# B-R-P/NMSLIB-ZIG

Hardware: AMD Instinct MI355X
Metric: queries/sec @ recall@10, 1M x 128-D L2, batch=1024; HBM GB/s vs peak (higher is better)
Workload: dtype f16+f32

## Files before the change

### nmslib_zig_amd/csrc/kernels/bf_kernels.hip

```cpp
#include <cstdio>
#include <type_traits>
#include <vector>
#include <cstdlib>

#include "common_dev.hpp"
#include "kernels.hpp"

namespace gfxknn {

enum BfMode : int { BF_L2 = 0, BF_DOT = 1, BF_COS = 2, BF_L1 = 3, BF_LINF = 4, BF_COSC = 5, BF_L2D = 6 };

struct BfArgs {
    const float* base;
    const float* aux;
    const float* qaux;
    int aux_stride;
    const float* queries;
    u64* cand;
    int* cand_cnt;
    uint32_t* gthr;
    uint32_t* gq;
    int xj, xm;
    int n, ldb, nqt, nsplit, rows_per_split, kprime, cap;
    int kcs;
// ... 772 lines not shown
        else asm volatile("s_waitcnt vmcnt(0)\n\ts_barrier" ::: "memory");
    }
    if (nstages > 0 && !(a.dbg & 1)) {
        if (a.xj > 0 && !(a.dbg & 256)) exchange_counted();
        finish_stage(true);
    }
    if (h == 0) a.cand_cnt[(size_t)qidx * a.nsplit + split] = mycnt;
}

__device__ __forceinline__ uint32_t hit_mask_f32(const f32x16& c, float t) {
    typedef float f32x2 __attribute__((ext_vector_type(2)));
    uint32_t m = 0u;
    const f32x2 tt = {t, t};
#pragma unroll
    for (int i0 = 0; i0 < 16; i0 += 8) {
        f32x2 d[4];
#pragma unroll
        for (int j = 0; j < 4; ++j) d[j] = f32x2{c[i0 + 2 * j], c[i0 + 2 * j + 1]} - tt;
        asm volatile("" : "+v"(d[0]), "+v"(d[1]), "+v"(d[2]), "+v"(d[3]));
#pragma unroll
        for (int j = 0; j < 4; ++j) {
            m = __builtin_amdgcn_alignbit(m, __float_as_uint(d[j][0]), 31);
            m = __builtin_amdgcn_alignbit(m, __float_as_uint(d[j][1]), 31);
        }
    }
    return ~m & 0xffffu;
}
__device__ __forceinline__ uint32_t hit_mask_i32(const i32x16& c, int t) {
    uint32_t m = 0u;
#pragma unroll
    for (int i = 0; i < 16; ++i) m = __builtin_amdgcn_alignbit(m, (uint32_t)(c[i] - t), 31);
    return ~m & 0xffffu;
}
__device__ __forceinline__ void scan_gather_entries(u64* keys, const int* offs, const uint32_t* list, int q, int nl, int caph,
                                                    int tps, int tid, int nthreads) {
    for (int s = tid; s < nl; s += nthreads) {
        const int len = offs[s + 1] - offs[s];
        if (len == 0) continue;
        const uint32_t* e = list + (size_t)q * caph * nl + s;
        const uint32_t row_base = (uint32_t)(s >> 1) * (uint32_t)tps * BF_BN + 4u * (s & 1);
        uint32_t pre[4];
#pragma unroll
        for (int i = 0; i < 4; ++i) pre[i] = (i < len && i < caph) ? e[(size_t)i * nl] : 0u;
        int j = 0;
        auto expand = [&](const uint32_t ent) __attribute__((always_inline)) {
            uint32_t m = ent & 0xffffu;
            const uint32_t r0 = row_base + (ent >> 16) * 32u;
            while (m && j < len) {
                const int bit = 31 - __builtin_clz(m);
                m &= ~(1u << bit);
                const int reg = 15 - bit;
                keys[offs[s] + j++] = (u64)(r0 + (reg & 3) + 8 * (reg >> 2));
            }
        };
#pragma unroll
        for (int i = 0; i < 4; ++i)
            if (i < caph && j < len) expand(pre[i]);
        for (int i = 4; i < caph && j < len; ++i) expand(e[(size_t)i * nl]);
    }
}

struct BfScanArgs {
    const uint8_t* base_i8;
    const int32_t* auxh;
    const uint8_t* queries;
    const int* thr;
    uint32_t* list;
    int* list_cnt;
    int n, nqt, nsplit, tps, caph;
    int tile_stride;
    int* top8;
};

template <int QG, bool SAMPLE>
__global__ __launch_bounds__(256, 2) void bf_scan_u8_kernel(BfScanArgs a) {
    extern __shared__ __attribute__((aligned(16))) char smem[];
    const int tid = threadIdx.x, lane = tid & 63, wave = tid >> 6;
    const int h = lane >> 5, l31 = lane & 31;
    const int b = blockIdx.x;
    const int xcd = b & 7, rest = b >> 3;
    const int qt = rest % a.nqt;
    const int split = (rest / a.nqt) * 8 + xcd;
    if (split >= a.nsplit) return;

    constexpr int kGroup = 4, kRing = 2 * kGroup, kAuxRing = 8, kTileBytes = BF_BN * 128;
    char* ring = smem;
    int* auxr = reinterpret_cast<int*>(ring + kRing * kTileBytes);

    const int tstr = SAMPLE ? a.tile_stride : 1;
    const int tiles_all = (a.n + BF_BN - 1) / BF_BN;
    const int stiles_all = (tiles_all + tstr - 1) / tstr;
// ... 1073 lines not shown
        const float need = 2.1f * e1;
        uint32_t best = 0u;
#pragma unroll
        for (int i = 0; i < NPER; ++i) {
            const float v = ord_f32(key[i]);
            const bool c = key[i] != 0u && key[i] <= T && v > -INFINITY && t3 - v >= need;
            best = c && key[i] > best ? key[i] : best;
        }
#pragma unroll
        for (int o = 32; o > 0; o >>= 1) {
            const uint32_t other = (uint32_t)__shfl_xor((int)best, o, 64);
            best = other > best ? other : best;
        }
        ok = false;
        if (best != 0u) {
            int above = 0;
#pragma unroll
            for (int i = 0; i < NPER; ++i) above += __popcll(__builtin_amdgcn_ballot_w64(key[i] > best));
            const int jmax = rcap < total ? rcap : total;
            const int j = best == T ? r : above + 1;
            if (j <= jmax) {
                t1 = ord_f32(best);
                ok = true;
            }
        }
    }
    if (lane == 0) {
        thr3[q] = (t3 - 1.02f * e1) / unit;
        thr1[q] = force_precise == 2 ? INFINITY : t1;
        if (!ok) atomicOr(&precise[q / group_q], 1);
    }
}

struct RerankListF32Args {
    const float* base;
    const float* queries;
    const uint32_t* list;
    const int* list_cnt;
    const int32_t* ext_ids;
    int32_t* out_ids;
    float* out_dists;
    int32_t* out_cnt;
    int* tile_fail;
    int n, k, nsplit, caph, p2max, fail_queries, space, dim, ldb;
    int tps;
    const float* queries_sel;
    const float* thr;
    const float* thr1;
    const int* precise;
    int no_split;
    float bmax;
    float bres;
    float scale, scale_q, bres16;
    int sel_dim, sel_ld;
    const float* qaux;
    unsigned long long* prof;
};

__global__ __launch_bounds__(256) void bf_rerank_f32_list_kernel(RerankListF32Args a) {
    const unsigned long long t0 = a.prof ? wall_clock64() : 0;
    auto lap = [&](int i) __attribute__((always_inline)) {
        if (a.prof && threadIdx.x == 0) atomicAdd(&a.prof[i], wall_clock64() - t0);
    };
    extern __shared__ __attribute__((aligned(16))) char smem[];
    u64* keys = reinterpret_cast<u64*>(smem);
    int* offs = reinterpret_cast<int*>(keys + a.p2max);
    __shared__ int s_over, s_split;
    __shared__ float s_qn2, s_e1, s_thr;
    const int q = blockIdx.x, tid = threadIdx.x, lane = tid & 63, wave = tid >> 6;
    const int nl = 2 * a.nsplit;
    if (tid == 0) s_over = 0;
    __syncthreads();
    if (tid < 64) {
        const int per = (nl + 63) / 64;
        int sum = 0, over = 0;
        for (int i = 0; i < per; ++i) {
            const int s = tid * per + i;
            if (s < nl) {
                const int c = a.list_cnt[(size_t)q * nl + s];
                over |= c > a.caph;
                sum += c < a.caph ? c : a.caph;
            }
        }
        int incl = sum;
#pragma unroll
        for (int o = 1; o < 64; o <<= 1) {
            const int v = __shfl_up(incl, o, 64);
            if (tid >= o) incl += v;
        }
        int run = incl - sum;
        for (int i = 0; i < per; ++i) {
// ... 41 lines not shown
    if (a.prof && tid == 0) {
        atomicAdd(&a.prof[8], (unsigned long long)total);
        atomicAdd(&a.prof[9], (unsigned long long)P);
        atomicAdd(&a.prof[10], 1ull);
    }
    const float* qq = a.queries + (size_t)q * a.ldb;
    const int sub = lane & 15, rg = lane >> 4;
    if (a.dim <= 128) {
        float qv[8];
        bool ok[8];
    #pragma unroll
        for (int c = 0; c < 8; ++c) {
            const int d = sub + 16 * c;
            ok[c] = d < a.dim;
            qv[c] = ok[c] ? qq[d] : 0.f;
        }
        constexpr int kU = 4;
        for (int j0 = wave * (4 * kU); j0 < total; j0 += 16 * kU) {
            uint32_t pos[kU];
            float xv[kU][8];
    #pragma unroll
            for (int u = 0; u < kU; ++u) {
                const int j = j0 + 4 * u + rg;
                pos[u] = (uint32_t)keys[j < total ? j : total - 1];
                const float* row = a.base + (size_t)pos[u] * a.ldb + sub;
    #pragma unroll
                for (int c = 0; c < 8; ++c) xv[u][c] = ok[c] ? row[16 * c] : 0.f;
            }
            __builtin_amdgcn_wave_barrier();
    #pragma unroll
            for (int u = 0; u < kU; ++u) {
                float p0[4], p1[4], p2[4];
    #pragma unroll
                for (int v = 0; v < 4; ++v) {
                    p0[v] = p1[v] = p2[v] = 0.f;
    #pragma unroll
                    for (int c = 0; c < 2; ++c) {
                        if (64 * c >= a.dim) continue;
                        const float x = xv[u][v + 4 * c], y = qv[v + 4 * c];
                        if (a.space == SP_L2) {
                            const float t = x - y;
                            p0[v] = fmaf(t, t, p0[v]);
                        } else {
                            p0[v] = fmaf(x, y, p0[v]);
                            if (a.space != SP_NEGDOT) {
                                p1[v] = fmaf(x, x, p1[v]);
                                p2[v] = fmaf(y, y, p2[v]);
                            }
                        }
                    }
                }
                auto tree = [&](const float* p) __attribute__((always_inline)) -> float {
                    float s = (p[0] + p[2]) + (p[1] + p[3]);
    #pragma unroll
                    for (int o = 8; o > 0; o >>= 1) s += __shfl_xor(s, o, 64);
                    return s;
                };
                const float s0 = tree(p0);
                float d;
                if (a.space == SP_L2) d = sqrtf(s0);
                else if (a.space == SP_NEGDOT) d = -s0;
                else {
                    const float sim = normdot_finish(s0, tree(p1), tree(p2));
                    d = a.space == SP_ANGULAR ? acosf(sim) : fmaxf(0.0f, 1.0f - sim);
                }
                const int j = j0 + 4 * u + rg;
                if (sub == 0 && j < total) keys[j] = ((u64)f32_ord(d) << 32) | pos[u];
            }
        }
    } else {
        const int nstep = (a.dim + 63) >> 6;
        for (int j0 = wave * 16; j0 < total; j0 += 64) {
            uint32_t pos[4];
            const float* rowp[4];
    #pragma unroll
            for (int u = 0; u < 4; ++u) {
                const int j = j0 + 4 * u + rg;
                pos[u] = (uint32_t)keys[j < total ? j : total - 1];
                rowp[u] = a.base + (size_t)pos[u] * a.ldb + sub;
            }
            float p0[4][4], p1[4][4], p2[4][4];
    #pragma unroll
            for (int u = 0; u < 4; ++u)
    #pragma unroll
                for (int v = 0; v < 4; ++v) p0[u][v] = p1[u][v] = p2[u][v] = 0.f;
            for (int c0 = 0; c0 < nstep; c0 += 2) {
                float xv[4][8], qv[8];
                bool ok[8];
    #pragma unroll
                for (int c = 0; c < 8; ++c) {
                    const int d = sub + 16 * (c & 3) + 64 * (c0 + (c >> 2));
                    ok[c] = d < a.dim;
                    qv[c] = ok[c] ? qq[d] : 0.f;
    #pragma unroll
                    for (int u = 0; u < 4; ++u) xv[u][c] = ok[c] ? rowp[u][16 * (c & 3) + 64 * (c0 + (c >> 2))] : 0.f;
                }
    #pragma unroll
                for (int u = 0; u < 4; ++u) {
    #pragma unroll
                    for (int v = 0; v < 4; ++v) {
    #pragma unroll
                        for (int c = 0; c < 2; ++c) {
                            if (64 * (c0 + c) >= a.dim) continue;
                            const float x = xv[u][v + 4 * c], y = qv[v + 4 * c];
                            if (a.space == SP_L2) {
                                const float t = x - y;
                                p0[u][v] = fmaf(t, t, p0[u][v]);
                            } else {
                                p0[u][v] = fmaf(x, y, p0[u][v]);
                                if (a.space != SP_NEGDOT) {
                                    p1[u][v] = fmaf(x, x, p1[u][v]);
                                    p2[u][v] = fmaf(y, y, p2[u][v]);
                                }
                            }
                        }
                    }
                }
            }
            __builtin_amdgcn_wave_barrier();
    #pragma unroll
            for (int u = 0; u < 4; ++u) {
                auto tree = [&](const float* p) __attribute__((always_inline)) -> float {
                    float s = (p[0] + p[2]) + (p[1] + p[3]);
    #pragma unroll
                    for (int o = 8; o > 0; o >>= 1) s += __shfl_xor(s, o, 64);
                    return s;
                };
                const float s0 = tree(p0[u]);
                float d;
                if (a.space == SP_L2) d = sqrtf(s0);
                else if (a.space == SP_NEGDOT) d = -s0;
                else {
                    const float sim = normdot_finish(s0, tree(p1[u]), tree(p2[u]));
                    d = a.space == SP_ANGULAR ? acosf(sim) : fmaxf(0.0f, 1.0f - sim);
                }
                const int j = j0 + 4 * u + rg;
                if (sub == 0 && j < total) keys[j] = ((u64)f32_ord(d) << 32) | pos[u];
            }
        }
    }
    __syncthreads();
    lap(2);
    if (total <= 512 && a.k <= 32) {
        __shared__ u64 s_head[128];
        const int e0 = wave * 128 + 2 * lane;
        u64 k0 = e0 < total ? keys[e0] : ~0ull, k1 = e0 + 1 < total ? keys[e0 + 1] : ~0ull;
        wave_sort128_u64(k0, k1, lane);
        if (lane < 16) {
            s_head[wave * 32 + 2 * lane] = k0;
            s_head[wave * 32 + 2 * lane + 1] = k1;
        }
        __syncthreads();
        if (wave == 0) {
            k0 = s_head[2 * lane];
            k1 = s_head[2 * lane + 1];
            wave_sort128_u64(k0, k1, lane);
            if (lane < 16) {
                keys[2 * lane] = k0;
                keys[2 * lane + 1] = k1;
            }
        }
        __syncthreads();
    } else {
        for (int i = total + tid; i < P; i += blockDim.x) keys[i] = ~0ull;
        __syncthreads();
        block_bitonic_u64_asc(keys, P, tid, blockDim.x);
    }
    lap(3);
    const int found = total < a.k ? total : a.k;
    if (total < a.n) {
        const bool split_product = s_split != 0;
        if (tid == 0) {
            const float qn2 = s_qn2, qn = sqrtf(qn2);
            const float dk = ord_f32((uint32_t)(keys[found - 1] >> 32));
            float sk, e, extra = 0.f;
            if (a.qaux) {
                const float sh = sinf(0.5f * dk);
                const float omc = a.space == SP_ANGULAR ? 2.0f * sh * sh : dk;
                const float qnorm = a.qaux[(size_t)q * 4 + 2];
                sk = -omc * qnorm;
                e = 6.1036e-5f * qn * a.bmax;
                extra = 1e-6f * qn * a.bmax + 2e-6f * qnorm;
            } else if (a.space == SP_L2) {
                sk = 0.5f * (qn2 - dk * dk);
                e = 6.1036e-5f * qn * a.bmax;
            } else if (a.space == SP_NEGDOT) {
                sk = -dk;
                e = 6.1036e-5f * qn * a.bmax;
            } else {
                sk = (a.space == SP_ANGULAR ? cosf(dk) : 1.0f - dk) * qn;
                e = 6.1036e-5f * qn;
            }
            const float t = s_thr;
            if (!split_product) {
                const float unit = a.scale * a.scale_q;
                sk *= unit;
                extra *= unit;
                e = s_e1;
            }
            e += extra + 1e-6f * (fabsf(sk) + fabsf(t));
            if (!(sk - t >= e)) atomicOr(&a.tile_fail[q / a.fail_queries], 1);
        }
    }
    lap(4);
    for (int i = tid; i < a.k; i += blockDim.x) {
        int32_t id = -1;
        float d = INFINITY;
        if (i < found) {
            const u64 key = keys[i];
            const uint32_t pos = (uint32_t)key;
            id = a.ext_ids ? a.ext_ids[pos] : (int32_t)pos;
            d = ord_f32((uint32_t)(key >> 32));
        }
        a.out_ids[(size_t)q * a.k + i] = id;
        a.out_dists[(size_t)q * a.k + i] = d;
    }
    if (tid == 0 && a.out_cnt) a.out_cnt[q] = found;
    lap(5);
}

__global__ void row_maxnorm_kernel(const float* rows, int n, int ld, int dim, int relative, unsigned* out_bits, float scale16) {
    const int lane = threadIdx.x & 63;
    const int wpb = blockDim.x >> 6;
    float mb = 0.f, mr = 0.f, ma = 0.f, mh = 0.f;
    for (int row = blockIdx.x * wpb + (threadIdx.x >> 6); row < n; row += gridDim.x * wpb) {
        const float* p = rows + (size_t)row * ld;
        float s = 0.f, r = 0.f, rh = 0.f;
        for (int d = lane; d < dim; d += 64) {
            const float v = p[d], w = v - (float)(__bf16)v;
            const float vs = scale16 * v, wh = vs - (float)(_Float16)vs;
            s = fmaf(v, v, s);
            r = fmaf(w, w, r);
            rh = fmaf(wh, wh, rh);
            ma = fmaxf(ma, fabsf(v));
        }
        s = wave_sum(s);
        r = wave_sum(r);
        rh = wave_sum(rh);
        const float nb = sqrtf(s), nr = sqrtf(r), nh = sqrtf(rh);
        mb = fmaxf(mb, nb);
        mr = fmaxf(mr, relative ? (nb > 0.f ? nr / nb : 0.f) : nr);
        mh = fmaxf(mh, relative ? (nb > 0.f ? nh / nb : 0.f) : nh);
    }
    ma = wave_max(ma);
    if (lane == 0) {
        atomicMax(out_bits, __float_as_uint(mb));
        atomicMax(out_bits + 1, __float_as_uint(mr));
        atomicMax(out_bits + 2, __float_as_uint(ma));
        atomicMax(out_bits + 3, __float_as_uint(mh));
    }
}
// ... 904 lines not shown
    f.qg = nq >= 1024 ? 2 : 1;
    if (const char* e = getenv("NMSLIB_GPU_F32_QG")) f.qg = atoi(e) == 2 ? 2 : (atoi(e) == 1 ? 1 : f.qg);
    if (f.kch > 1) f.qg = 1;
    const int tq = f.kch > 1 ? 128 : 256 * f.qg;
    f.tq = tq;
    f.qpad = (nq + tq - 1) / tq * tq;
    f.nqt = f.qpad / tq;
    f.stride = 16;
    if (const char* e = getenv("NMSLIB_GPU_SAMPLE_STRIDE")) f.stride = atoi(e) > 0 ? atoi(e) : 16;
    const int kp = k + (k / 8 > 4 ? k / 8 : 4);
    const double kf = (double)kp / f.stride;
    f.r = (int)(1.6 * kf + 3.0 * sqrt(kf) + 3.0 + 0.999);
    f.rcap = 4 * f.r + 32;
    f.force_precise = false;
    if (const char* e = getenv("NMSLIB_GPU_F32_TERMS")) f.force_precise = atoi(e) == 3;
    const int tiles_all = (n + BF_BN - 1) / BF_BN;
    int ns = (256 + f.nqt - 1) / f.nqt;
    if (ns > tiles_all / 16) ns = tiles_all / 16;
    if (ns > 256) ns = 256;
    ns = (ns + 7) / 8 * 8;
    if (ns < 8) ns = 8;
    while ((tiles_all + ns - 1) / ns > 32768) ns += 8;
    f.nsplit = ns;
    f.tps = (tiles_all + ns - 1) / ns;
    const double mean_half = (double)f.rcap * f.stride / (2.0 * ns);
    int caph = 8;
    while (caph < 3.0 * mean_half + 8.0) caph <<= 1;
    f.caph = caph;
    f.p2max = host_next_pow2((int)(2.5 * f.rcap * f.stride) + 64);
    if (f.p2max > 2 * ns * caph) f.p2max = host_next_pow2(2 * ns * caph);
    f.lds_scan = 4 * 2 * BF_BN * 256 + 8 * BF_BN * 4 + 64;
    f.lds_scan1 = 9 * BF_BN * 256 + 16 * BF_BN * 4 + 64;
    f.lds_rerank = (size_t)f.p2max * 8 + (2 * (size_t)ns + 1) * 4 + 16;
    const int stiles = (tiles_all + f.stride - 1) / f.stride;
    const int s_nqt = f.qpad / (f.kch > 1 ? 128 : 256);
    int nss = (256 + s_nqt - 1) / s_nqt;
    if (nss > stiles / 16) nss = stiles / 16;
    if (nss > 64) nss = 64;
    nss = (nss + 7) / 8 * 8;
    if (nss < 8) nss = 8;
    f.s_nsplit = nss;
    f.s_tps = (stiles + nss - 1) / nss;
    f.lds_thr = (size_t)host_next_pow2(nss * 2 * 8) * 8 + 16;
    f.fallback = bf_make_plan(n, dim_rows, nq, k, false, tq);
    if (f.kch > 1) f.force_precise = false;
    return f;
}

hipError_t launch_row_maxnorm(const float* rows, int n, int ld, int dim, bool relative_residual, float* out, hipStream_t s,
                              float scale16) {
    hipError_t e = hipMemsetAsync(out, 0, 16, s);
    if (e != hipSuccess || n == 0) return e;
    int grid = (n + 3) / 4;
    if (grid > 4096) grid = 4096;
    hipLaunchKernelGGL(row_maxnorm_kernel, dim3(grid), dim3(256), 0, s, rows, n, ld, dim, relative_residual ? 1 : 0,
                       reinterpret_cast<unsigned*>(out), scale16);
    return hipGetLastError();
}

hipError_t launch_split_bf16(const float* src, int rows, int rows_pad, int ld, int dim, void* hi, void* lo,
                             const float* aux, float aux_pad, float* auxp, hipStream_t s, int dp, void* h16, float scale,
                             float* auxp16, float aux16_mul) {
    const size_t total = (size_t)rows_pad * dp;
    if (total == 0) return hipSuccess;
    size_t grid = (total + 255) / 256;
    if (grid > 16384) grid = 16384;
// ... 147 lines not shown
    r.out_dists = out_dists;
    r.out_cnt = out_cnt;
    r.tile_fail = tile_fail;
    r.n = n;
    r.k = k;
    r.nsplit = f.nsplit;
    r.caph = f.caph;
    r.tps = f.tps;
    r.p2max = f.p2max;
    r.fail_queries = f.tq;
    r.no_split = f.kch > 1 ? 1 : 0;
    r.space = space;
    r.dim = dim;
    r.ldb = ldb;
    r.queries_sel = queries_sel;
    r.sel_dim = sdim;
    r.sel_ld = sld;
    r.scale = h16.scale;
    r.scale_q = h16.scale_q;
    r.bres16 = h16.bres16;
    r.qaux = f.cosc ? qaux_cosc : nullptr;
    r.thr = thr;
    r.thr1 = thr1;
    r.precise = precise;
    r.bmax = bmax;
    r.bres = bres;
    static const int dbg_prof = getenv("NMSLIB_GPU_DEBUG") ? atoi(getenv("NMSLIB_GPU_DEBUG")) : 0;
    static unsigned long long* d_prof = nullptr;
    if (dbg_prof & 4096) {
        if (!d_prof) (void)hipMalloc(&d_prof, 16 * 8);
        (void)hipMemsetAsync(d_prof, 0, 16 * 8, s);
        r.prof = d_prof;
    }
    e = hipFuncSetAttribute(reinterpret_cast<const void*>(bf_rerank_f32_list_kernel),
                            hipFuncAttributeMaxDynamicSharedMemorySize, (int)f.lds_rerank);
    if (e != hipSuccess) return e;
    hipLaunchKernelGGL(bf_rerank_f32_list_kernel, dim3(nq), dim3(256), f.lds_rerank, s, r);
    e = hipGetLastError();
    if (e != hipSuccess) return e;
    if (dbg_prof & 4096) {
        unsigned long long h[16];
        (void)hipStreamSynchronize(s);
        (void)hipMemcpy(h, d_prof, sizeof(h), hipMemcpyDeviceToHost);
        const double wg = h[10] ? (double)h[10] : 1.0;
        fprintf(stderr, "[rerank f32 list] workgroups %llu rows/query %.1f P %.1f | us since start: prefix %.2f gather %.2f distances %.2f "
                "sort %.2f proof %.2f out %.2f\n", h[10], h[8] / wg, h[9] / wg, h[0] / wg / 100, h[1] / wg / 100, h[2] / wg / 100,
                h[3] / wg / 100, h[4] / wg / 100, h[5] / wg / 100);
    }
    {
        static const int dbg = getenv("NMSLIB_GPU_DEBUG") ? atoi(getenv("NMSLIB_GPU_DEBUG")) : 0;
        if (dbg & 2048) {
            (void)hipStreamSynchronize(s);
            auto sum = [&](const void* d, size_t bytes) -> unsigned long long {
                std::vector<uint32_t> h(bytes / 4);
                (void)hipMemcpy(h.data(), d, bytes, hipMemcpyDeviceToHost);
                unsigned long long x = 1469598103934665603ull;
                for (uint32_t v : h) x = (x ^ v) * 1099511628211ull;
                return x;
            };
            std::vector<int> cnt((size_t)f.qpad * f.nsplit * 2);
            (void)hipMemcpy(cnt.data(), list_cnt, cnt.size() * 4, hipMemcpyDeviceToHost);
            std::vector<uint32_t> lst((size_t)f.qpad * f.nsplit * 2 * f.caph);
            (void)hipMemcpy(lst.data(), list, lst.size() * 4, hipMemcpyDeviceToHost);
            unsigned long long lx = 1469598103934665603ull;
            long long rows = 0;
            const size_t nl = (size_t)f.nsplit * 2;
            for (size_t i = 0; i < cnt.size(); ++i) {
                rows += cnt[i];
                int have = 0;
                for (int j = 0; j < f.caph && have < cnt[i]; ++j) {
                    const uint32_t e = lst[((i / nl) * f.caph + j) * nl + i % nl];
                    lx = (lx ^ e) * 1099511628211ull;
                    have += __builtin_popcount(e & 0xffffu);
// ... 113 lines not shown
```

### nmslib_zig_amd/csrc/kernels/kernels.hpp

```cpp
#pragma once
#include <hip/hip_runtime_api.h>
#include <stddef.h>
#include <stdint.h>

namespace gfxknn {

enum SpaceCode : int {
    SP_L2 = 0,
    SP_L1 = 1,
    SP_LINF = 2,
    SP_COSINE = 3,
    SP_ANGULAR = 4,
    SP_NEGDOT = 5,
    SP_L2SQR_SIFT = 6,
    SP_L2SQR = 7,
    SP_NORMCOS = 8,
    SP_QNORM_NEGDOT = 9,
    SP_LEVEN = 10,
    SP_BIT_HAMMING = 11,
};

constexpr int BF_TQ = 128;
constexpr int BF_BN = 64;
constexpr int BF_KC = 128;
// ... 53 lines not shown
    BfPlan fallback;
};
inline size_t bf_u8_top8_elems(const BfU8Fast& f) { return (size_t)f.qpad * f.s_nsplit * 2 * 8; }
BfU8Fast bf_u8_fast_plan(int n, int nq, int k);
inline size_t bf_u8_list_elems(const BfU8Fast& f) { return (size_t)f.qpad * f.nsplit * 2 * f.caph; }
inline size_t bf_u8_listcnt_elems(const BfU8Fast& f) { return (size_t)f.qpad * f.nsplit * 2; }
hipError_t launch_bf_u8_fast(const BfU8Fast& f, int n, int nq, int k, const uint8_t* base_u8, const uint8_t* base_i8,
                             const int32_t* aux, const int32_t* auxh, const uint8_t* queries_padded,
                             int* top8, unsigned long long* cand_fb, int* cnt_fb,
                             int* thr, uint32_t* list, int* list_cnt, int* tile_fail, const int32_t* ext_ids,
                             int32_t* out_ids, float* out_dists, int32_t* out_cnt, hipEvent_t scan_begin,
                             hipEvent_t scan_end, hipStream_t s, const uint8_t* queries_raw);

hipError_t launch_bf_select_f32_ex(const BfPlan& p, int space, const float* base, const float* aux,
                                   const float* queries_padded, const float* qaux_cosc, unsigned long long* cand,
                                   int* cand_cnt, const int* tile_fail, int fail_group, hipStream_t s, bool cleared = false);

struct BfF32Fast {
    bool use;
    int mode;
    int qg;
    bool cosc;
    int sel_dim;
    int kch;
    int dp;
    int tq;
    int qpad, nqt;
    int stride, r;
    int rcap;
    bool force_precise;
    int nsplit, tps, caph, p2max;
    int s_nsplit, s_tps;
    size_t lds_scan, lds_scan1, lds_thr, lds_rerank;
    BfPlan fallback;
};
BfF32Fast bf_f32_fast_plan(int n, int dim, int nq, int k, int space, bool cosine_centred);
inline size_t bf_f32_thr_bytes(const BfF32Fast& f) { return (size_t)f.qpad * 8 + (size_t)f.nqt * 8 + 64; }
inline size_t bf_f32_list_elems(const BfF32Fast& f) { return (size_t)f.qpad * f.nsplit * 2 * f.caph; }
inline size_t bf_f32_listcnt_elems(const BfF32Fast& f) { return (size_t)f.qpad * f.nsplit * 2; }
inline size_t bf_f32_top8_elems(const BfF32Fast& f) { return (size_t)f.qpad * f.s_nsplit * 2 * 8; }
inline int bf_f32_rows_padded(int n) { return (n + BF_BN - 1) / BF_BN * BF_BN + BF_BN; }
hipError_t launch_row_maxnorm(const float* rows, int n, int ld, int dim, bool relative_residual, float* out, hipStream_t s,
                              float scale16 = 0.f);
hipError_t launch_split_bf16(const float* src, int rows, int rows_pad, int ld, int dim, void* hi, void* lo,
                             const float* aux, float aux_pad, float* auxp, hipStream_t s, int dp = 128, void* h16 = nullptr,
                             float scale = 1.f, float* auxp16 = nullptr, float aux16_mul = 1.f);
struct BfF16Side {
    const void* base_h16;
    const float* auxp16;
    void* q_h16;
    float scale;
    float bres16;
    float scale_q;
};
hipError_t launch_bf_f32_fast(const BfF32Fast& f, int space, int n, int dim, int ldb, int nq, int k, const float* base_orig,
                              const float* sel_rows, const float* aux, const void* base_hi, const void* base_lo,
                              const float* auxp, float bmax, float bres, const float* queries_orig, const float* queries_sel,
                              void* q_hi, void* q_lo, float* top8, unsigned long long* cand_fb, int* cnt_fb, float* thr,
                              uint32_t* list, int* list_cnt, int* tile_fail, int* flags_fb, const int32_t* ext_ids, int32_t* out_ids,
                              float* out_dists, int32_t* out_cnt, hipEvent_t scan_begin, hipEvent_t scan_end,
                              hipStream_t s, const float* queries_raw = nullptr, float* queries_pad_out = nullptr,
                              const float* qaux_cosc = nullptr, const float* queries_centred = nullptr, int sel_ld = 0,
                              const BfF16Side& h16 = BfF16Side{});
hipError_t launch_row_aug_cosc(const float* orig, const float* centred, int n, int ldb, int dim, double mu_norm, float lambda,
                               float* out, int ldo, int* zero_rows, hipStream_t s);
hipError_t launch_query_aug_cosc(const float* centred, const float* qaux, int nq, int qpad, int ldb, int dim, float lambda,
// ... 233 lines not shown
```

Before: 2.864 million.

## Add persistent software-pipelined f32 rerank kernel overlapping next query's list fetch

Adds a persistent rerank kernel launched with about one workgroup per CU that loops over queries. It double-buffers per-query state in LDS, prefetching the next query's candidate list, counts and thresholds while the current query's rows are scored. Row loads are vectorised to float4 and prefetched one iteration ahead, and a wider shuffle reduction is used. Small candidate lists are expanded straight from registers, and the old kernel is kept as fallback when kch>1, k>32 or the split count is large. It trades launch parallelism and higher LDS use per workgroup for hiding global-memory latency.

Measured after the change: 2.540 million. -11.3%, worse.

```diff
diff --git a/nmslib_zig_amd/csrc/kernels/bf_kernels.hip b/nmslib_zig_amd/csrc/kernels/bf_kernels.hip
--- a/nmslib_zig_amd/csrc/kernels/bf_kernels.hip
+++ b/nmslib_zig_amd/csrc/kernels/bf_kernels.hip
@@ -828,31 +828,37 @@
     for (int i = 0; i < 16; ++i) m = __builtin_amdgcn_alignbit(m, (uint32_t)(c[i] - t), 31);
     return ~m & 0xffffu;
 }
+__device__ __forceinline__ void scan_expand_list(u64* keys, const int* offs, const uint32_t* e, int s, int nl, int caph, int tps,
+                                                 const uint32_t (&pre)[4]) {
+    const int len = offs[s + 1] - offs[s];
+    if (len == 0) return;
+    const uint32_t row_base = (uint32_t)(s >> 1) * (uint32_t)tps * BF_BN + 4u * (s & 1);
+    int j = 0;
+    auto expand = [&](const uint32_t ent) __attribute__((always_inline)) {
+        uint32_t m = ent & 0xffffu;
+        const uint32_t r0 = row_base + (ent >> 16) * 32u;
+        while (m && j < len) {
+            const int bit = 31 - __builtin_clz(m);
+            m &= ~(1u << bit);
+            const int reg = 15 - bit;
+            keys[offs[s] + j++] = (u64)(r0 + (reg & 3) + 8 * (reg >> 2));
+        }
+    };
+#pragma unroll
+    for (int i = 0; i < 4; ++i)
+        if (i < caph && j < len) expand(pre[i]);
+    for (int i = 4; i < caph && j < len; ++i) expand(e[(size_t)i * nl]);
+}
 __device__ __forceinline__ void scan_gather_entries(u64* keys, const int* offs, const uint32_t* list, int q, int nl, int caph,
                                                     int tps, int tid, int nthreads) {
     for (int s = tid; s < nl; s += nthreads) {
         const int len = offs[s + 1] - offs[s];
         if (len == 0) continue;
         const uint32_t* e = list + (size_t)q * caph * nl + s;
-        const uint32_t row_base = (uint32_t)(s >> 1) * (uint32_t)tps * BF_BN + 4u * (s & 1);
         uint32_t pre[4];
 #pragma unroll
         for (int i = 0; i < 4; ++i) pre[i] = (i < len && i < caph) ? e[(size_t)i * nl] : 0u;
-        int j = 0;
-        auto expand = [&](const uint32_t ent) __attribute__((always_inline)) {
-            uint32_t m = ent & 0xffffu;
-            const uint32_t r0 = row_base + (ent >> 16) * 32u;
-            while (m && j < len) {
-                const int bit = 31 - __builtin_clz(m);
-                m &= ~(1u << bit);
-                const int reg = 15 - bit;
-                keys[offs[s] + j++] = (u64)(r0 + (reg & 3) + 8 * (reg >> 2));
-            }
-        };
-#pragma unroll
-        for (int i = 0; i < 4; ++i)
-            if (i < caph && j < len) expand(pre[i]);
-        for (int i = 4; i < caph && j < len; ++i) expand(e[(size_t)i * nl]);
+        scan_expand_list(keys, offs, e, s, nl, caph, tps, pre);
     }
 }
 
@@ -1992,6 +1998,51 @@
     }
 }
 
+__device__ __forceinline__ void rerank_row_chains(int space, int dim, int step0, const float (&xv)[8], const float (&qv)[8],
+                                                  float (&p0)[4], float (&p1)[4], float (&p2)[4]) {
+#pragma unroll
+    for (int v = 0; v < 4; ++v) {
+#pragma unroll
+        for (int c = 0; c < 2; ++c) {
+            if (64 * (step0 + c) >= dim) continue;
+            const float x = xv[v + 4 * c], y = qv[v + 4 * c];
+            if (space == SP_L2) {
+                const float t = x - y;
+                p0[v] = fmaf(t, t, p0[v]);
+            } else {
+                p0[v] = fmaf(x, y, p0[v]);
+                if (space != SP_NEGDOT) {
+                    p1[v] = fmaf(x, x, p1[v]);
+                    p2[v] = fmaf(y, y, p2[v]);
+                }
+            }
+        }
+    }
+}
+template <bool WIDE>
+__device__ __forceinline__ float rerank_row_tree(const float (&p)[4]) {
+    if (WIDE) {
+        float s[4] = {p[0], p[1], p[2], p[3]};
+#pragma unroll
+        for (int o = 8; o > 0; o >>= 1)
+#pragma unroll
+            for (int v = 0; v < 4; ++v) s[v] += __shfl_xor(s[v], o, 64);
+        return (s[0] + s[2]) + (s[1] + s[3]);
+    }
+    float s = (p[0] + p[2]) + (p[1] + p[3]);
+#pragma unroll
+    for (int o = 8; o > 0; o >>= 1) s += __shfl_xor(s, o, 64);
+    return s;
+}
+template <bool WIDE>
+__device__ __forceinline__ float rerank_row_finish(int space, const float (&p0)[4], const float (&p1)[4], const float (&p2)[4]) {
+    const float s0 = rerank_row_tree<WIDE>(p0);
+    if (space == SP_L2) return sqrtf(s0);
+    if (space == SP_NEGDOT) return -s0;
+    const float sim = normdot_finish(s0, rerank_row_tree<WIDE>(p1), rerank_row_tree<WIDE>(p2));
+    return space == SP_ANGULAR ? acosf(sim) : fmaxf(0.0f, 1.0f - sim);
+}
+
 struct RerankListF32Args {
     const float* base;
     const float* queries;
@@ -2017,6 +2068,89 @@
     unsigned long long* prof;
 };
 
+template <class Lap>
+__device__ __forceinline__ void rerank_list_f32_finish(const RerankListF32Args& a, int q, u64* keys, int total, int split,
+                                                       float qn2, float e1, float thr, Lap lap) {
+    const int tid = threadIdx.x, lane = tid & 63, wave = tid >> 6;
+    const int P = next_pow2(total < 2 ? 2 : total);
+    if (total <= 512 && a.k <= 32) {
+        __shared__ u64 s_head[128];
+        const int e0 = wave * 128 + 2 * lane;
+        u64 k0 = e0 < total ? keys[e0] : ~0ull, k1 = e0 + 1 < total ? keys[e0 + 1] : ~0ull;
+        wave_sort128_u64(k0, k1, lane);
+        if (lane < 16) {
+            s_head[wave * 32 + 2 * lane] = k0;
+            s_head[wave * 32 + 2 * lane + 1] = k1;
+        }
+        __syncthreads();
+        if (wave == 0) {
+            k0 = s_head[2 * lane];
+            k1 = s_head[2 * lane + 1];
+            wave_sort128_u64(k0, k1, lane);
+            if (lane < 16) {
+                keys[2 * lane] = k0;
+                keys[2 * lane + 1] = k1;
+            }
+        }
+        __syncthreads();
+    } else {
+        for (int i = total + tid; i < P; i += blockDim.x) keys[i] = ~0ull;
+        __syncthreads();
+        block_bitonic_u64_asc(keys, P, tid, blockDim.x);
+    }
+    lap(3);
+    const int found = total < a.k ? total : a.k;
+    if (total < a.n) {
+        const bool split_product = split != 0;
+        if (tid == 0) {
+            const float qn = sqrtf(qn2);
+            const float dk = ord_f32((uint32_t)(keys[found - 1] >> 32));
+            float sk, e, extra = 0.f;
+            if (a.qaux) {
+                const float sh = sinf(0.5f * dk);
+                const float omc = a.space == SP_ANGULAR ? 2.0f * sh * sh : dk;
+                const float qnorm = a.qaux[(size_t)q * 4 + 2];
+                sk = -omc * qnorm;
+                e = 6.1036e-5f * qn * a.bmax;
+                extra = 1e-6f * qn * a.bmax + 2e-6f * qnorm;
+            } else if (a.space == SP_L2) {
+                sk = 0.5f * (qn2 - dk * dk);
+                e = 6.1036e-5f * qn * a.bmax;
+            } else if (a.space == SP_NEGDOT) {
+                sk = -dk;
+                e = 6.1036e-5f * qn * a.bmax;
+            } else {
+                sk = (a.space == SP_ANGULAR ? cosf(dk) : 1.0f - dk) * qn;
+                e = 6.1036e-5f * qn;
+            }
+            const float t = thr;
+            if (!split_product) {
+                const float unit = a.scale * a.scale_q;
+                sk *= unit;
+                extra *= unit;
+                e = e1;
+            }
+            e += extra + 1e-6f * (fabsf(sk) + fabsf(t));
+            if (!(sk - t >= e)) atomicOr(&a.tile_fail[q / a.fail_queries], 1);
+        }
+    }
+    lap(4);
+    for (int i = tid; i < a.k; i += blockDim.x) {
+        int32_t id = -1;
+        float d = INFINITY;
+        if (i < found) {
+            const u64 key = keys[i];
+            const uint32_t pos = (uint32_t)key;
+            id = a.ext_ids ? a.ext_ids[pos] : (int32_t)pos;
+            d = ord_f32((uint32_t)(key >> 32));
+        }
+        a.out_ids[(size_t)q * a.k + i] = id;
+        a.out_dists[(size_t)q * a.k + i] = d;
+    }
+    if (tid == 0 && a.out_cnt) a.out_cnt[q] = found;
+    lap(5);
+}
+
 __global__ __launch_bounds__(256) void bf_rerank_f32_list_kernel(RerankListF32Args a) {
     const unsigned long long t0 = a.prof ? wall_clock64() : 0;
     auto lap = [&](int i) __attribute__((always_inline)) {
@@ -2124,38 +2258,9 @@
             for (int u = 0; u < kU; ++u) {
                 float p0[4], p1[4], p2[4];
     #pragma unroll
-                for (int v = 0; v < 4; ++v) {
-                    p0[v] = p1[v] = p2[v] = 0.f;
-    #pragma unroll
-                    for (int c = 0; c < 2; ++c) {
-                        if (64 * c >= a.dim) continue;
-                        const float x = xv[u][v + 4 * c], y = qv[v + 4 * c];
-                        if (a.space == SP_L2) {
-                            const float t = x - y;
-                            p0[v] = fmaf(t, t, p0[v]);
-                        } else {
-                            p0[v] = fmaf(x, y, p0[v]);
-                            if (a.space != SP_NEGDOT) {
-                                p1[v] = fmaf(x, x, p1[v]);
-                                p2[v] = fmaf(y, y, p2[v]);
-                            }
-                        }
-                    }
-                }
-                auto tree = [&](const float* p) __attribute__((always_inline)) -> float {
-                    float s = (p[0] + p[2]) + (p[1] + p[3]);
-    #pragma unroll
-                    for (int o = 8; o > 0; o >>= 1) s += __shfl_xor(s, o, 64);
-                    return s;
-                };
-                const float s0 = tree(p0);
-                float d;
-                if (a.space == SP_L2) d = sqrtf(s0);
-                else if (a.space == SP_NEGDOT) d = -s0;
-                else {
-                    const float sim = normdot_finish(s0, tree(p1), tree(p2));
-                    d = a.space == SP_ANGULAR ? acosf(sim) : fmaxf(0.0f, 1.0f - sim);
-                }
+                for (int v = 0; v < 4; ++v) p0[v] = p1[v] = p2[v] = 0.f;
+                rerank_row_chains(a.space, a.dim, 0, xv[u], qv, p0, p1, p2);
+                const float d = rerank_row_finish<false>(a.space, p0, p1, p2);
                 const int j = j0 + 4 * u + rg;
                 if (sub == 0 && j < total) keys[j] = ((u64)f32_ord(d) << 32) | pos[u];
             }
@@ -2188,44 +2293,12 @@
                     for (int u = 0; u < 4; ++u) xv[u][c] = ok[c] ? rowp[u][16 * (c & 3) + 64 * (c0 + (c >> 2))] : 0.f;
                 }
     #pragma unroll
-                for (int u = 0; u < 4; ++u) {
-    #pragma unroll
-                    for (int v = 0; v < 4; ++v) {
-    #pragma unroll
-                        for (int c = 0; c < 2; ++c) {
-                            if (64 * (c0 + c) >= a.dim) continue;
-                            const float x = xv[u][v + 4 * c], y = qv[v + 4 * c];
-                            if (a.space == SP_L2) {
-                                const float t = x - y;
-                                p0[u][v] = fmaf(t, t, p0[u][v]);
-                            } else {
-                                p0[u][v] = fmaf(x, y, p0[u][v]);
-                                if (a.space != SP_NEGDOT) {
-                                    p1[u][v] = fmaf(x, x, p1[u][v]);
-                                    p2[u][v] = fmaf(y, y, p2[u][v]);
-                                }
-                            }
-                        }
-                    }
-                }
+                for (int u = 0; u < 4; ++u) rerank_row_chains(a.space, a.dim, c0, xv[u], qv, p0[u], p1[u], p2[u]);
             }
             __builtin_amdgcn_wave_barrier();
     #pragma unroll
             for (int u = 0; u < 4; ++u) {
-                auto tree = [&](const float* p) __attribute__((always_inline)) -> float {
-                    float s = (p[0] + p[2]) + (p[1] + p[3]);
-    #pragma unroll
-                    for (int o = 8; o > 0; o >>= 1) s += __shfl_xor(s, o, 64);
-                    return s;
-                };
-                const float s0 = tree(p0[u]);
-                float d;
-                if (a.space == SP_L2) d = sqrtf(s0);
-                else if (a.space == SP_NEGDOT) d = -s0;
-                else {
-                    const float sim = normdot_finish(s0, tree(p1[u]), tree(p2[u]));
-                    d = a.space == SP_ANGULAR ? acosf(sim) : fmaxf(0.0f, 1.0f - sim);
-                }
+                const float d = rerank_row_finish<false>(a.space, p0[u], p1[u], p2[u]);
                 const int j = j0 + 4 * u + rg;
                 if (sub == 0 && j < total) keys[j] = ((u64)f32_ord(d) << 32) | pos[u];
             }
@@ -2233,82 +2306,201 @@
     }
     __syncthreads();
     lap(2);
-    if (total <= 512 && a.k <= 32) {
-        __shared__ u64 s_head[128];
-        const int e0 = wave * 128 + 2 * lane;
-        u64 k0 = e0 < total ? keys[e0] : ~0ull, k1 = e0 + 1 < total ? keys[e0 + 1] : ~0ull;
-        wave_sort128_u64(k0, k1, lane);
-        if (lane < 16) {
-            s_head[wave * 32 + 2 * lane] = k0;
-            s_head[wave * 32 + 2 * lane + 1] = k1;
+    rerank_list_f32_finish(a, q, keys, total, s_split, s_qn2, s_e1, s_thr, lap);
+}
+
+constexpr int kRerankPipeCap = 512;
+__global__ __launch_bounds__(256) void bf_rerank_f32_list_pipe_kernel(RerankListF32Args a, int nq) {
+    typedef float f32x4 __attribute__((ext_vector_type(4)));
+    extern __shared__ __attribute__((aligned(16))) char smem[];
+    const int nl = 2 * a.nsplit;
+    u64* keys_small = reinterpret_cast<u64*>(smem);
+    u64* keys_big = keys_small + 2 * kRerankPipeCap;
+    int* offs_all = reinterpret_cast<int*>(keys_big + a.p2max);
+    float* sq_all = reinterpret_cast<float*>(offs_all + 2 * (nl + 1));
+    __shared__ int s_state[2], s_total[2], s_split[2];
+    __shared__ float s_qn2[2], s_e1[2], s_thr[2];
+    const int tid = threadIdx.x, lane = tid & 63, wave = tid >> 6;
+    const int sub = lane & 15, rg = lane >> 4;
+    const int need = a.k < a.n ? a.k : a.n;
+    const int want = need + (a.k / 8 > 4 ? a.k / 8 : 4) < a.n ? need + (a.k / 8 > 4 ? a.k / 8 : 4) : a.n;
+    bool ok[8];
+#pragma unroll
+    for (int c = 0; c < 8; ++c) ok[c] = 64 * (c >> 2) + 4 * sub + (c & 3) < a.dim;
+
+    int f_cnt[2] = {0, 0};
+    uint32_t f_pre[2][4] = {};
+    float f_sq = 0.f, f_thr = 0.f, f_thr1 = 0.f, f_qflag = 1.f;
+    int f_precise = 0;
+    uint32_t r_pos[4] = {};
+    f32x4 r_x[4][2] = {};
+    f32x4 r_q[2] = {};
+
+    auto front_request = [&](int qn) __attribute__((always_inline)) {
+#pragma unroll
+        for (int u = 0; u < 2; ++u) {
+            const int s = tid + 256 * u;
+            if (s < nl) {
+                f_cnt[u] = a.list_cnt[(size_t)qn * nl + s];
+                const uint32_t* e = a.list + (size_t)qn * a.caph * nl + s;
+#pragma unroll
+                for (int i = 0; i < 4; ++i) f_pre[u][i] = i < a.caph ? e[(size_t)i * nl] : 0u;
+            }
+        }
+        if (tid < a.sel_dim) f_sq = a.queries_sel[(size_t)qn * a.sel_ld + tid];
+        f_precise = a.precise[qn / a.fail_queries];
+        f_thr = a.thr[qn];
+        f_thr1 = a.thr1[qn];
+        if (a.qaux) f_qflag = a.qaux[(size_t)qn * 4 + 3];
+    };
+    auto rows_request = [&](const u64* keys, int total, int j0, uint32_t (&pos)[4], f32x4 (&x)[4][2]) __attribute__((always_inline)) {
+#pragma unroll
+        for (int u = 0; u < 4; ++u) {
+            const int j = j0 + 4 * u + rg;
+            pos[u] = (uint32_t)keys[j < total ? j : total - 1];
+            const float* row = a.base + (size_t)pos[u] * a.ldb + 4 * sub;
+#pragma unroll
+            for (int h = 0; h < 2; ++h)
+                x[u][h] = ok[4 * h] ? *reinterpret_cast<const f32x4*>(row + 64 * h) : f32x4{0.f, 0.f, 0.f, 0.f};
+        }
+    };
+    auto query_request = [&](int q, f32x4 (&y)[2]) __attribute__((always_inline)) {
+        const float* qq = a.queries + (size_t)q * a.ldb + 4 * sub;
+#pragma unroll
+        for (int h = 0; h < 2; ++h) y[h] = ok[4 * h] ? *reinterpret_cast<const f32x4*>(qq + 64 * h) : f32x4{0.f, 0.f, 0.f, 0.f};
+    };
+    auto front_finish = [&](int qn, int t) __attribute__((always_inline)) {
+        int* offs = offs_all + t * (nl + 1);
+        float* sq = sq_all + t * a.sel_dim;
+        int over = 0;
+#pragma unroll
+        for (int u = 0; u < 2; ++u) {
+            const int s = tid + 256 * u;
+            if (s < nl) {
+                over |= f_cnt[u] > a.caph;
+                offs[s + 1] = f_cnt[u] < a.caph ? f_cnt[u] : a.caph;
+            }
+        }
+        if (tid < a.sel_dim) sq[tid] = f_sq;
+        const int over_any = __syncthreads_or(over);
+        if (wave == 0) {
+            const int per = (nl + 63) / 64;
+            int sum = 0;
+            for (int i = 0; i < per; ++i) {
+                const int s = lane * per + i;
+                if (s < nl) sum += offs[s + 1];
+            }
+            int incl = sum;
+#pragma unroll
+            for (int o = 1; o < 64; o <<= 1) {
+                const int v = __shfl_up(incl, o, 64);
+                if (lane >= o) incl += v;
+            }
+            int run = incl - sum;
+            for (int i = 0; i < per; ++i) {
+                const int s = lane * per + i;
+                if (s < nl) {
+                    run += offs[s + 1];
+                    offs[s + 1] = run;
+                }
+            }
+            if (lane == 0) offs[0] = 0;
+            if (lane == 63) {
+                const int total = incl;
+                int state = total <= kRerankPipeCap ? 1 : 2;
+                if ((a.no_split && f_precise != 0) ||
+                    (a.qaux && f_qflag == 0.f) ||
+                    over_any || total < want || total > a.p2max) {
+                    atomicOr(&a.tile_fail[qn / a.fail_queries], 1);
+                    state = 0;
+                }
+                s_state[t] = state;
+                s_total[t] = total;
+            }
+        } else if (wave == 1) {
+            const bool split_product = f_precise != 0;
+            float ss = 0.f;
+            for (int d = lane; d < a.sel_dim; d += 64) ss = fmaf(sq[d], sq[d], ss);
+            ss = wave_sum(ss);
+            const float e1 = split_product ? 0.f : one_product_error(sq, a.sel_dim, lane, a.scale * (a.space == SP_L2 || a.space == SP_NEGDOT || a.qaux ? a.bmax : 1.0f), a.bres16, a.scale_q);
+            if (lane == 0) {
+                s_qn2[t] = ss;
+                s_e1[t] = e1;
+                s_split[t] = split_product ? 1 : 0;
+                s_thr[t] = split_product ? f_thr : f_thr1;
+            }
         }
         __syncthreads();
-        if (wave == 0) {
-            k0 = s_head[2 * lane];
-            k1 = s_head[2 * lane + 1];
-            wave_sort128_u64(k0, k1, lane);
-            if (lane < 16) {
-                keys[2 * lane] = k0;
-                keys[2 * lane + 1] = k1;
+        if (s_state[t] == 1) {
+            u64* keys = keys_small + t * kRerankPipeCap;
+#pragma unroll
+            for (int u = 0; u < 2; ++u) {
+                const int s = tid + 256 * u;
+                if (s < nl) scan_expand_list(keys, offs, a.list + (size_t)qn * a.caph * nl + s, s, nl, a.caph, a.tps, f_pre[u]);
+            }
+            __syncthreads();
+            query_request(qn, r_q);
+            rows_request(keys, s_total[t], wave * 16, r_pos, r_x);
+        }
+    };
+
+    int q = blockIdx.x, slot = 0;
+    if (q < nq) {
+        front_request(q);
+        front_finish(q, 0);
+    }
+    for (; q < nq; q += gridDim.x, slot ^= 1) {
+        const int qn = q + gridDim.x;
+        const int state = s_state[slot], total = s_total[slot];
+        u64* keys = state == 2 ? keys_big : keys_small + slot * kRerankPipeCap;
+        if (state == 2) {
+            __syncthreads();
+            scan_gather_entries(keys, offs_all + slot * (nl + 1), a.list, q, nl, a.caph, a.tps, tid, blockDim.x);
+            __syncthreads();
+        }
+        if (qn < nq) front_request(qn);
+        if (state != 0) {
+            if (state == 2) {
+                query_request(q, r_q);
+                rows_request(keys, total, wave * 16, r_pos, r_x);
+            }
+            float qv[8];
+#pragma unroll
+            for (int c = 0; c < 8; ++c) qv[c] = ok[c] ? r_q[c >> 2][c & 3] : 0.f;
+            for (int j0 = wave * 16; j0 < total; j0 += 64) {
+                uint32_t n_pos[4] = {};
+                f32x4 n_x[4][2] = {};
+                const bool more = j0 + 64 < total;
+                if (more) rows_request(keys, total, j0 + 64, n_pos, n_x);
+                __builtin_amdgcn_wave_barrier();
+#pragma unroll
+                for (int u = 0; u < 4; ++u) {
+                    float xv[8], p0[4], p1[4], p2[4];
+#pragma unroll
+                    for (int c = 0; c < 8; ++c) xv[c] = ok[c] ? r_x[u][c >> 2][c & 3] : 0.f;
+#pragma unroll
+                    for (int v = 0; v < 4; ++v) p0[v] = p1[v] = p2[v] = 0.f;
+                    rerank_row_chains(a.space, a.dim, 0, xv, qv, p0, p1, p2);
+                    const float d = rerank_row_finish<true>(a.space, p0, p1, p2);
+                    const int j = j0 + 4 * u + rg;
+                    if (sub == 0 && j < total) keys[j] = ((u64)f32_ord(d) << 32) | r_pos[u];
+                }
+                if (more) {
+#pragma unroll
+                    for (int u = 0; u < 4; ++u) {
+                        r_pos[u] = n_pos[u];
+                        r_x[u][0] = n_x[u][0];
+                        r_x[u][1] = n_x[u][1];
+                    }
+                }
             }
         }
         __syncthreads();
-    } else {
-        for (int i = total + tid; i < P; i += blockDim.x) keys[i] = ~0ull;
-        __syncthreads();
-        block_bitonic_u64_asc(keys, P, tid, blockDim.x);
-    }
-    lap(3);
-    const int found = total < a.k ? total : a.k;
-    if (total < a.n) {
-        const bool split_product = s_split != 0;
-        if (tid == 0) {
-            const float qn2 = s_qn2, qn = sqrtf(qn2);
-            const float dk = ord_f32((uint32_t)(keys[found - 1] >> 32));
-            float sk, e, extra = 0.f;
-            if (a.qaux) {
-                const float sh = sinf(0.5f * dk);
-                const float omc = a.space == SP_ANGULAR ? 2.0f * sh * sh : dk;
-                const float qnorm = a.qaux[(size_t)q * 4 + 2];
-                sk = -omc * qnorm;
-                e = 6.1036e-5f * qn * a.bmax;
-                extra = 1e-6f * qn * a.bmax + 2e-6f * qnorm;
-            } else if (a.space == SP_L2) {
-                sk = 0.5f * (qn2 - dk * dk);
-                e = 6.1036e-5f * qn * a.bmax;
-            } else if (a.space == SP_NEGDOT) {
-                sk = -dk;
-                e = 6.1036e-5f * qn * a.bmax;
-            } else {
-                sk = (a.space == SP_ANGULAR ? cosf(dk) : 1.0f - dk) * qn;
-                e = 6.1036e-5f * qn;
-            }
-            const float t = s_thr;
-            if (!split_product) {
-                const float unit = a.scale * a.scale_q;
-                sk *= unit;
-                extra *= unit;
-                e = s_e1;
-            }
-            e += extra + 1e-6f * (fabsf(sk) + fabsf(t));
-            if (!(sk - t >= e)) atomicOr(&a.tile_fail[q / a.fail_queries], 1);
-        }
-    }
-    lap(4);
-    for (int i = tid; i < a.k; i += blockDim.x) {
-        int32_t id = -1;
-        float d = INFINITY;
-        if (i < found) {
-            const u64 key = keys[i];
-            const uint32_t pos = (uint32_t)key;
-            id = a.ext_ids ? a.ext_ids[pos] : (int32_t)pos;
-            d = ord_f32((uint32_t)(key >> 32));
-        }
-        a.out_ids[(size_t)q * a.k + i] = id;
-        a.out_dists[(size_t)q * a.k + i] = d;
-    }
-    if (tid == 0 && a.out_cnt) a.out_cnt[q] = found;
-    lap(5);
+        const int split = s_split[slot];
+        const float qn2 = s_qn2[slot], e1 = s_e1[slot], thr = s_thr[slot];
+        if (qn < nq) front_finish(qn, slot ^ 1);
+        if (state != 0) rerank_list_f32_finish(a, q, keys, total, split, qn2, e1, thr, [](int) {});
+    }
 }
 
 __global__ void row_maxnorm_kernel(const float* rows, int n, int ld, int dim, int relative, unsigned* out_bits, float scale16) {
@@ -3279,6 +3471,9 @@
     f.lds_scan = 4 * 2 * BF_BN * 256 + 8 * BF_BN * 4 + 64;
     f.lds_scan1 = 9 * BF_BN * 256 + 16 * BF_BN * 4 + 64;
     f.lds_rerank = (size_t)f.p2max * 8 + (2 * (size_t)ns + 1) * 4 + 16;
+    f.rerank_pipe = f.kch == 1 && k <= 32 && 2 * ns <= 512;
+    if (const char* e = getenv("NMSLIB_GPU_RERANK_LIST")) f.rerank_pipe = f.rerank_pipe && atoi(e) != 0;
+    f.lds_rerank_pipe = (2 * (size_t)kRerankPipeCap + f.p2max) * 8 + 2 * (2 * (size_t)ns + 1) * 4 + 2 * (size_t)f.sel_dim * 4 + 16;
     const int stiles = (tiles_all + f.stride - 1) / f.stride;
     const int s_nqt = f.qpad / (f.kch > 1 ? 128 : 256);
     int nss = (256 + s_nqt - 1) / s_nqt;
@@ -3492,13 +3687,29 @@
         (void)hipMemsetAsync(d_prof, 0, 16 * 8, s);
         r.prof = d_prof;
     }
-    e = hipFuncSetAttribute(reinterpret_cast<const void*>(bf_rerank_f32_list_kernel),
-                            hipFuncAttributeMaxDynamicSharedMemorySize, (int)f.lds_rerank);
-    if (e != hipSuccess) return e;
-    hipLaunchKernelGGL(bf_rerank_f32_list_kernel, dim3(nq), dim3(256), f.lds_rerank, s, r);
+    if (f.rerank_pipe) {
+        static const int cus = [] {
+            int dev = 0, n = 0;
+            if (hipGetDevice(&dev) != hipSuccess || hipDeviceGetAttribute(&n, hipDeviceAttributeMultiprocessorCount, dev) != hipSuccess) n = 0;
+            return n > 0 ? n : 256;
+        }();
+        int per_cu = 1;
+        if (const char* w = getenv("NMSLIB_GPU_RERANK_WGS")) per_cu = atoi(w) >= 1 && atoi(w) <= 3 ? atoi(w) : per_cu;
+        const int grid_pipe = nq < per_cu * cus ? nq : per_cu * cus;
+        r.prof = nullptr;
+        e = hipFuncSetAttribute(reinterpret_cast<const void*>(bf_rerank_f32_list_pipe_kernel),
+                                hipFuncAttributeMaxDynamicSharedMemorySize, (int)f.lds_rerank_pipe);
+        if (e != hipSuccess) return e;
+        hipLaunchKernelGGL(bf_rerank_f32_list_pipe_kernel, dim3(grid_pipe), dim3(256), f.lds_rerank_pipe, s, r, nq);
+    } else {
+        e = hipFuncSetAttribute(reinterpret_cast<const void*>(bf_rerank_f32_list_kernel),
+                                hipFuncAttributeMaxDynamicSharedMemorySize, (int)f.lds_rerank);
+        if (e != hipSuccess) return e;
+        hipLaunchKernelGGL(bf_rerank_f32_list_kernel, dim3(nq), dim3(256), f.lds_rerank, s, r);
+    }
     e = hipGetLastError();
     if (e != hipSuccess) return e;
-    if (dbg_prof & 4096) {
+    if ((dbg_prof & 4096) && !f.rerank_pipe) {
         unsigned long long h[16];
         (void)hipStreamSynchronize(s);
         (void)hipMemcpy(h, d_prof, sizeof(h), hipMemcpyDeviceToHost);
diff --git a/nmslib_zig_amd/csrc/kernels/kernels.hpp b/nmslib_zig_amd/csrc/kernels/kernels.hpp
--- a/nmslib_zig_amd/csrc/kernels/kernels.hpp
+++ b/nmslib_zig_amd/csrc/kernels/kernels.hpp
@@ -109,6 +109,8 @@
     int nsplit, tps, caph, p2max;
     int s_nsplit, s_tps;
     size_t lds_scan, lds_scan1, lds_thr, lds_rerank;
+    bool rerank_pipe;
+    size_t lds_rerank_pipe;
     BfPlan fallback;
 };
 BfF32Fast bf_f32_fast_plan(int n, int dim, int nq, int k, int space, bool cosine_centred);
```
